# sunilsarolkarcds/ISL-SignLanguage-Translation

Measured on AMD Instinct MI355X. Metric: frames/sec body_25 368×656 fwd+NMS+PAF at 1/8 MI355X; conv MFMA util %, higher is better.
Workload: dtype fp32 (split-fp16 x3 MFMA, fp32 accumulate)

## Files before the change

### isl-signlanguage-translation_amd/csrc/wino_f16.hip

```cpp
#include <algorithm>
#include <cstdlib>
#include <type_traits>

#include "internal.h"

namespace isl {
namespace {

typedef _Float16 f16x8 __attribute__((ext_vector_type(8)));
typedef _Float16 f16x2 __attribute__((ext_vector_type(2)));
typedef float f32x2 __attribute__((ext_vector_type(2)));
typedef float f32x4 __attribute__((ext_vector_type(4)));
typedef float f32x16 __attribute__((ext_vector_type(16)));
typedef unsigned u32x4 __attribute__((ext_vector_type(4)));

struct W2Args {
  const float* in;
  float* out;
  const f16x8* upk;
  const float* bias;
  const float* slope;
  int* range_flag;
  long long in_fs, in_chs, out_fs, out_chs;
  float wscale_inv;
  int in_pad, out_pad, H, W, TH, TW, pairs, cin_chunks, co_blocks, bpf, act, nblocks;
};

constexpr int RS = 34;
constexpr int QS = 6 * 2 * RS;
constexpr int HS = 13 * 64;
constexpr int BUF = 32 * 64;

__device__ __forceinline__ void split_dw(const f32x4& v, unsigned& h01, unsigned& h23, unsigned& l01, unsigned& l23) {
  asm("v_cvt_pk_f16_f32 %0, %1, %2" : "=v"(h01) : "v"(v.x), "v"(v.y));
  asm("v_cvt_pk_f16_f32 %0, %1, %2" : "=v"(h23) : "v"(v.z), "v"(v.w));
  asm("v_fma_mixlo_f16 %0, %1, -1.0, %2 op_sel_hi:[1,0,0]" : "=v"(l01) : "v"(h01), "v"(v.x));
  asm("v_fma_mixhi_f16 %0, %1, -1.0, %2 op_sel:[1,0,0] op_sel_hi:[1,0,0]" : "+v"(l01) : "v"(h01), "v"(v.y));
  asm("v_fma_mixlo_f16 %0, %1, -1.0, %2 op_sel_hi:[1,0,0]" : "=v"(l23) : "v"(h23), "v"(v.z));
  asm("v_fma_mixhi_f16 %0, %1, -1.0, %2 op_sel:[1,0,0] op_sel_hi:[1,0,0]" : "+v"(l23) : "v"(h23), "v"(v.w));
}

template <int ABL>
__global__ void __launch_bounds__(512, 1) wino_f16(W2Args a) {
  __shared__ f32x4 smem[8192 + 32];

  int bid = blockIdx.x;
  {
    const int nb = a.nblocks, q = nb >> 3, r = nb & 7, xcd = bid & 7, k = bid >> 3;
    bid = (xcd < r ? xcd * (q + 1) : r * (q + 1) + (xcd - r) * q) + k;
  }
  const int co_b = bid % a.co_blocks;
  const int rest = bid / a.co_blocks;
  const int fb = rest % a.bpf;
  const int n = rest / a.bpf;

  const int tid = threadIdx.x, lane = tid & 63, h = lane >> 5, l32 = lane & 31;
  const int w = __builtin_amdgcn_readfirstlane(tid >> 6);

  if (tid < 64) {
    float* eb = (float*)(smem + 8192);
    eb[tid] = a.bias[co_b * 64 + tid];
    eb[64 + tid] = a.act == ACT_PRELU ? a.slope[co_b * 64 + tid] : 0.f;
  }

  const int BW = 2 * a.TW, s0 = fb * 64;
  const int ba = s0 / BW, bb = (s0 + 63) / BW;
  const bool two = bb > ba;
  const int txlo0 = (s0 - ba * BW) >> 1;
  const int txhi0 = two ? a.TW - 1 : (s0 + 63 - ba * BW) >> 1;
  const int w0 = 2 * (txhi0 - txlo0 + 1) + 2;
  const int w1 = two ? 2 * (((s0 + 63 - bb * BW) >> 1) + 1) + 2 : 0;
  const int Hp = a.H + 2 * a.in_pad, Wp = a.W + 2 * a.in_pad;
  const float* in_f = a.in + (size_t)n * a.in_fs;

  int doff[4], dch[4];
#pragma unroll
  for (int e = 0; e < 4; ++e) {
    const int p = w + 8 * e;
    const int hp = p < 26 ? p / 13 : 0;
    const int u = (p - 13 * hp) * 64 + lane;
    int t = u / RS;
    const int hc = u - t * RS;
    const int par = t & 1;
    t >>= 1;
    const int row = t % 6;
    const int qq = t / 6;
    const int v = 2 * hc + par;
    const bool s1 = v >= w0;
    const int vl = s1 ? v - w0 : v;
    const bool ok = p < 26 && qq < 2 && vl < (s1 ? w1 : w0);
    const int band = s1 ? bb : ba, txlo = s1 ? 0 : txlo0;
    const int rp = min(4 * band - 1 + row + a.in_pad, Hp - 1);
    const int cp = min(2 * txlo - 1 + vl + a.in_pad, Wp - 1);
    doff[e] = ok ? (rp * Wp + cp) * 8 + qq * 4 : 0;
    dch[e] = __builtin_amdgcn_readfirstlane(hp);
  }

  const int wr = w >> 1, cpr = w & 1;
  const int ra = wr == 0 ? 0 : wr == 2 ? 2 : 1, rb = wr == 3 ? 3 : wr == 2 ? 1 : 2;
  const float sr = wr == 1 ? 1.f : -1.f, sz = cpr ? -1.f : 1.f;
  const f32x4 srv = f32x4{sr, sr, sr, sr}, szv = f32x4{sz, sz, sz, sz};
  const int cX = cpr ? 2 : 0, cY = cpr ? 1 : 2, cZ = cpr ? 3 : 1;
  auto toff = [&](int row, int col) { return (row * 2 + (col & 1)) * RS + (col >> 1); };
  const int to_aX = toff(ra, cX), to_aY = toff(ra, cY), to_aZ = toff(ra, cZ);
  const int to_bX = toff(rb, cX), to_bY = toff(rb, cY), to_bZ = toff(rb, cZ);
  int tb[2];
#pragma unroll
  for (int j = 0; j < 2; ++j) {
    const int s = s0 + 32 * j + l32;
    const int band = s / BW, u = s - band * BW, tx = u >> 1, typ = u & 1;
    const int hc0 = band > ba ? (w0 >> 1) + tx : tx - txlo0;
    tb[j] = h * HS + 2 * typ * 2 * RS + hc0;
  }

  const unsigned uvoff = (unsigned)lane * 16;
  auto load_a = [&](f16x8 (&A)[2][2][2], int k) __attribute__((always_inline)) {
    if constexpr ((ABL & 4) != 0) return;
    const f16x8* u0 = a.upk + ((size_t)(co_b * a.pairs + k) * 16 + 4 * wr + 2 * cpr) * 256;
    const f16x8* u1 = u0 + 256;
    asm volatile(
        "global_load_dwordx4 %0, %8, %9 offset:0\n\t"
        "global_load_dwordx4 %1, %8, %9 offset:1024\n\t"
        "global_load_dwordx4 %2, %8, %9 offset:2048\n\t"
        "global_load_dwordx4 %3, %8, %9 offset:3072\n\t"
        "global_load_dwordx4 %4, %8, %10 offset:0\n\t"
        "global_load_dwordx4 %5, %8, %10 offset:1024\n\t"
        "global_load_dwordx4 %6, %8, %10 offset:2048\n\t"
        "global_load_dwordx4 %7, %8, %10 offset:3072"
        : "=v"(A[0][0][0]), "=v"(A[0][0][1]), "=v"(A[0][1][0]), "=v"(A[0][1][1]), "=v"(A[1][0][0]),
          "=v"(A[1][0][1]), "=v"(A[1][1][0]), "=v"(A[1][1][1])
        : "v"(uvoff), "s"(u0), "s"(u1)
        : "memory");
  };
  auto dma = [&](int k, int sl) __attribute__((always_inline)) {
    if constexpr ((ABL & 8) != 0) return;
#pragma unroll
    for (int e = 0; e < 4; ++e) {
      const int ch = min(2 * k + dch[e], a.cin_chunks - 1);
      const float* src = in_f + (size_t)ch * a.in_chs;
      __builtin_amdgcn_global_load_lds((const void*)(src + doff[e]),
                                       (__attribute__((address_space(3))) void*)(smem + sl * BUF + (w + 8 * e) * 64),
                                       16, 0, 0);
    }
  };

  f32x16 acc[2][2][2];
#pragma unroll
  for (int x = 0; x < 2; ++x)
#pragma unroll
    for (int i = 0; i < 2; ++i)
#pragma unroll
      for (int j = 0; j < 2; ++j)
#pragma unroll
        for (int r = 0; r < 16; ++r) acc[x][i][j][r] = 0.f;

  auto compute = [&](const f16x8 (&A)[2][2][2], int sl) __attribute__((always_inline)) {
#pragma unroll
    for (int j = 0; j < 2; ++j) {
      int b = tb[j] + sl * BUF;
      asm volatile("" : "+v"(b));
      unsigned Bd[2][2][4];
      if constexpr ((ABL & 2) != 0) {
#pragma unroll
        for (int x = 0; x < 2; ++x)
#pragma unroll
          for (int hl = 0; hl < 2; ++hl)
#pragma unroll
            for (int d = 0; d < 4; ++d) Bd[x][hl][d] = 0x3c003c00u;
      } else {
        auto quad = [&](auto qc) __attribute__((always_inline)) {
          constexpr int Q = decltype(qc)::value;
          const f32x4 aX = smem[b + to_aX + Q * QS], aY = smem[b + to_aY + Q * QS], aZ = smem[b + to_aZ + Q * QS];
          const f32x4 bX = smem[b + to_bX + Q * QS], bY = smem[b + to_bY + Q * QS], bZ = smem[b + to_bZ + Q * QS];
          const f32x4 tX = __builtin_elementwise_fma(srv, bX, aX);
          const f32x4 tY = __builtin_elementwise_fma(srv, bY, aY);
          const f32x4 tZ = __builtin_elementwise_fma(srv, bZ, aZ);
          const f32x4 v0 = tX - tY;
          const f32x4 v1 = __builtin_elementwise_fma(szv, tZ, tY);
          split_dw(v0, Bd[0][0][2 * Q], Bd[0][0][2 * Q + 1], Bd[0][1][2 * Q], Bd[0][1][2 * Q + 1]);
          split_dw(v1, Bd[1][0][2 * Q], Bd[1][0][2 * Q + 1], Bd[1][1][2 * Q], Bd[1][1][2 * Q + 1]);
        };
        quad(std::integral_constant<int, 0>{});
        quad(std::integral_constant<int, 1>{});
      }
      f16x8 Bh[2], Bl[2];
#pragma unroll
      for (int x = 0; x < 2; ++x) {
        Bh[x] = __builtin_bit_cast(f16x8, u32x4{Bd[x][0][0], Bd[x][0][1], Bd[x][0][2], Bd[x][0][3]});
        Bl[x] = __builtin_bit_cast(f16x8, u32x4{Bd[x][1][0], Bd[x][1][1], Bd[x][1][2], Bd[x][1][3]});
      }
#pragma unroll
      for (int x = 0; x < 2; ++x)
#pragma unroll
        for (int i = 0; i < 2; ++i) {
          if constexpr ((ABL & 1) != 0) continue;
          acc[x][i][j] = __builtin_amdgcn_mfma_f32_32x32x16_f16(A[x][i][0], Bh[x], acc[x][i][j], 0, 0, 0);
          acc[x][i][j] = __builtin_amdgcn_mfma_f32_32x32x16_f16(A[x][i][0], Bl[x], acc[x][i][j], 0, 0, 0);
          acc[x][i][j] = __builtin_amdgcn_mfma_f32_32x32x16_f16(A[x][i][1], Bh[x], acc[x][i][j], 0, 0, 0);
        }
    }
  };

  f16x8 AS[2][2][2][2];
  load_a(AS[0], 0);
  dma(0, 0);
  dma(min(1, a.pairs - 1), 1);
  asm volatile("s_waitcnt vmcnt(4)" ::: "memory");
  __syncthreads();
  __builtin_amdgcn_sched_barrier(0);
  auto step = [&](int k, f16x8 (&A)[2][2][2], f16x8 (&An)[2][2][2]) __attribute__((always_inline)) {
    load_a(An, min(k + 1, a.pairs - 1));
    dma(min(k + 2, a.pairs - 1), (k + 2) % 3);
    __builtin_amdgcn_sched_barrier(0);
    if constexpr ((ABL & 4) == 0)
      asm volatile("s_waitcnt vmcnt(16)"
                   : "+v"(A[0][0][0]), "+v"(A[0][0][1]), "+v"(A[0][1][0]), "+v"(A[0][1][1]), "+v"(A[1][0][0]),
                     "+v"(A[1][0][1]), "+v"(A[1][1][0]), "+v"(A[1][1][1])
                   :
                   : "memory");
    compute(A, k % 3);
    __builtin_amdgcn_sched_barrier(0);
    asm volatile("s_waitcnt vmcnt(12) lgkmcnt(0)" ::: "memory");
    __builtin_amdgcn_s_barrier();
    __builtin_amdgcn_sched_barrier(0);
  };
  for (int k = 0; k < a.pairs; k += 2) {
    step(k, AS[0], AS[1]);
    if (k + 1 < a.pairs) step(k + 1, AS[1], AS[0]);
  }
  asm volatile("s_waitcnt vmcnt(0) lgkmcnt(0)"
               : "+v"(AS[0][0][0][0]), "+v"(AS[0][0][0][1]), "+v"(AS[0][0][1][0]), "+v"(AS[0][0][1][1]),
                 "+v"(AS[0][1][0][0]), "+v"(AS[0][1][0][1]), "+v"(AS[0][1][1][0]), "+v"(AS[0][1][1][1]),
                 "+v"(AS[1][0][0][0]), "+v"(AS[1][0][0][1]), "+v"(AS[1][0][1][0]), "+v"(AS[1][0][1][1]),
                 "+v"(AS[1][1][0][0]), "+v"(AS[1][1][0][1]), "+v"(AS[1][1][1][0]), "+v"(AS[1][1][1][1])
               :
               : "memory");
  __syncthreads();

  bool bad = false;
  if constexpr ((ABL & 16) != 0) {
    float sum = 0.f;
#pragma unroll
    for (int x = 0; x < 2; ++x)
#pragma unroll
      for (int i = 0; i < 2; ++i)
#pragma unroll
        for (int j = 0; j < 2; ++j)
#pragma unroll
          for (int r = 0; r < 16; ++r) sum += acc[x][i][j][r];
    if (sum == 1.2345f || bad) atomicOr(a.range_flag, 1);
    return;
  }
  f32x4* xm = smem;
  const float* eb = (const float*)(smem + 8192);
  const int Wo = a.W + 2 * a.out_pad;
  float* out_f = a.out + (size_t)n * a.out_fs;
  const int rn = tid & 31, rh = (tid >> 5) & 1, rq = (tid >> 6) & 3, rj = tid >> 8;
  const int rs = s0 + 32 * rj + rn, rband = rs / BW, ru = rs - rband * BW, rtx = ru >> 1, rty = 2 * rband + (ru & 1);
#pragma unroll
  for (int i = 0; i < 2; ++i) {
#pragma unroll
    for (int x = 0; x < 2; ++x)
#pragma unroll
      for (int j = 0; j < 2; ++j)
#pragma unroll
        for (int q = 0; q < 4; ++q)
          xm[((((2 * w + x) * 2 + j) * 4 + q) * 2 + h) * 32 + l32] =
              f32x4{acc[x][i][j][4 * q], acc[x][i][j][4 * q + 1], acc[x][i][j][4 * q + 2], acc[x][i][j][4 * q + 3]};
    __syncthreads();
    {
      const f32x4* mp = xm + ((rj * 4 + rq) * 2 + rh) * 32 + rn;
      f32x4 R0[4], R1[4];
#pragma unroll
      for (int c = 0; c < 4; ++c) {
        const f32x4 m0 = mp[(0 + c) * 512], m1 = mp[(4 + c) * 512], m2 = mp[(8 + c) * 512], m3 = mp[(12 + c) * 512];
        R0[c] = (m0 + m1) + m2;
        R1[c] = (m1 - m2) - m3;
      }
      f32x4 Y[2][2];
      Y[0][0] = (R0[0] + R0[1]) + R0[2];
      Y[0][1] = (R0[1] - R0[2]) - R0[3];
      Y[1][0] = (R1[0] + R1[1]) + R1[2];
      Y[1][1] = (R1[1] - R1[2]) - R1[3];
      const int cl = i * 32 + 8 * rq + 4 * rh, co = co_b * 64 + cl;
      const f32x4 bv = *(const f32x4*)(eb + cl);
      const f32x4 sl = *(const f32x4*)(eb + 64 + cl);
      if (rty < a.TH) {
        float* oc = out_f + (size_t)(co >> 3) * a.out_chs + (co & 7);
#pragma unroll
        for (int yy = 0; yy < 2; ++yy)
#pragma unroll
          for (int xx = 0; xx < 2; ++xx) {
            const int y = 2 * rty + yy, x = 2 * rtx + xx;
            if (y >= a.H || x >= a.W) continue;
            f32x4 v;
#pragma unroll
            for (int e = 0; e < 4; ++e) v[e] = Y[yy][xx][e] * a.wscale_inv + bv[e];
            if (a.act == ACT_RELU) {
#pragma unroll
              for (int e = 0; e < 4; ++e) v[e] = v[e] > 0.f ? v[e] : 0.f;
            } else if (a.act == ACT_PRELU) {
#pragma unroll
              for (int e = 0; e < 4; ++e) v[e] = v[e] >= 0.f ? v[e] : v[e] * sl[e];
            }
#pragma unroll
            for (int e = 0; e < 4; ++e) bad |= !(__builtin_fabsf(v[e]) < 65504.f);
            *(f32x4*)(oc + (size_t)((y + a.out_pad) * Wo + x + a.out_pad) * 8) = v;
          }
      }
    }
    __syncthreads();
  }
  if (bad) atomicOr(a.range_flag, 1);
}

int g_wino_blocks(const ConvLaunch& c, int* bpf) {
  const int TH = (c.H + 1) / 2, TW = (c.W + 1) / 2, nbands = (TH + 1) / 2;
  *bpf = (nbands * 2 * TW + 63) / 64;
  return c.n * *bpf * (c.cout / 64);
}

}

bool wino_f16_fits(const ConvLaunch& c) {
  return c.ks == 3 && c.in_pad >= 1 && c.cout % 64 == 0 && c.cout > 0 && !c.hpool && !c.vin && !c.fold &&
         c.cout7 == 0 && (c.W + 1) / 2 >= 32 && (long long)c.H * c.W > 1024 &&
         !((c.in_cs | c.in_coff | c.out_cs | c.out_coff) & 7) && (long long)(c.H + 2 * c.in_pad) * (c.W + 2 * c.in_pad) * 8 < (1ll << 30);
}

hipError_t launch_wino_f16(const ConvLaunch& c, hipStream_t s) {
  if (!wino_f16_fits(c)) { set_error("wino_f16: launch not eligible"); return hipErrorInvalidValue; }
  if (!c.wx3 || !c.range_flag) { set_error("wino_f16: split filters / range flag missing"); return hipErrorInvalidValue; }
  W2Args a{};
  a.in_chs = (long long)(c.H + 2 * c.in_pad) * (c.W + 2 * c.in_pad) * 8;
  a.out_chs = (long long)(c.H + 2 * c.out_pad) * (c.W + 2 * c.out_pad) * 8;
  a.in_fs = a.in_chs * (c.in_cs / 8);
  a.out_fs = a.out_chs * (c.out_cs / 8);
  a.in = c.in + (c.in_coff / 8) * a.in_chs;
  a.out = c.out + (c.out_coff / 8) * a.out_chs;
  a.upk = (const f16x8*)c.wx3;
  a.bias = c.bias;
  a.slope = c.slope;
  a.range_flag = c.range_flag;
  a.wscale_inv = c.wscale_inv;
  a.in_pad = c.in_pad;
  a.out_pad = c.out_pad;
  a.H = c.H;
  a.W = c.W;
  a.TH = (c.H + 1) / 2;
  a.TW = (c.W + 1) / 2;
  a.pairs = (c.cin_chunks + 1) / 2;
  a.cin_chunks = c.cin_chunks;
  a.co_blocks = c.cout / 64;
  a.act = c.act;
  const long long nb = g_wino_blocks(c, &a.bpf);
  if (nb <= 0 || nb > 0x7fffffff) { set_error("wino_f16: bad grid"); return hipErrorInvalidValue; }
  a.nblocks = (int)nb;
#ifdef ISLPOSE_DEV
  const int abl = getenv("ISLPOSE_W2_ABL") ? atoi(getenv("ISLPOSE_W2_ABL")) : 0;
  switch (abl) {
#define W2ABL(k) case k: hipLaunchKernelGGL(wino_f16<k>, dim3(a.nblocks), dim3(512), 0, s, a); return hipGetLastError();
    W2ABL(1) W2ABL(2) W2ABL(3) W2ABL(4) W2ABL(6) W2ABL(8) W2ABL(12) W2ABL(14) W2ABL(16) W2ABL(31)
#undef W2ABL
    default: break;
  }
#endif
  hipLaunchKernelGGL(wino_f16<0>, dim3(a.nblocks), dim3(512), 0, s, a);
  return hipGetLastError();
}

double wino_f16_mfma_flops(const ConvLaunch& c) {
  int bpf = 0;
  const double nb = g_wino_blocks(c, &bpf);
  return nb * 16.0 * 64 * 64 * 16.0 * ((c.cin_chunks + 1) / 2) * 2 * 3;
}

}
```

Measured before the change: 1291.

## Software-pipeline LDS reads of Winograd input tiles ahead of transform and MFMA

Adds a prefetching compute path that issues the ds_read_b128 loads for the next quad/column group through inline asm before the current group's input transform and MFMAs run. The first group's reads are hoisted to the start of each step, ahead of the global loads. The B-transform now uses packed v_pk_fma_f32 with scalar sign constants, and the DMA offsets become byte offsets. The goal is to hide LDS latency behind the arithmetic, at the cost of more registers and hand-placed waitcnt barriers that could stall or cause hazards. The prefetch variant becomes the default, and the old path stays reachable through an env var in dev builds.

```diff
diff --git a/isl-signlanguage-translation_amd/csrc/wino_f16.hip b/isl-signlanguage-translation_amd/csrc/wino_f16.hip
--- a/isl-signlanguage-translation_amd/csrc/wino_f16.hip
+++ b/isl-signlanguage-translation_amd/csrc/wino_f16.hip
@@ -40,7 +40,18 @@
   asm("v_fma_mixhi_f16 %0, %1, -1.0, %2 op_sel:[1,0,0] op_sel_hi:[1,0,0]" : "+v"(l23) : "v"(h23), "v"(v.w));
 }
 
-template <int ABL>
+struct W2Raw {
+  f32x4 aX, aY, aZ, bX, bY, bZ;
+};
+__device__ __forceinline__ f32x2 pk_fma_s(unsigned long long s, f32x2 b, f32x2 a) {
+  f32x2 d;
+  asm("v_pk_fma_f32 %0, %1, %2, %3" : "=v"(d) : "s"(s), "v"(b), "v"(a));
+  return d;
+}
+__device__ __forceinline__ f32x2 lo2(const f32x4& v) { return f32x2{v.x, v.y}; }
+__device__ __forceinline__ f32x2 hi2(const f32x4& v) { return f32x2{v.z, v.w}; }
+
+template <int ABL, int PF>
 __global__ void __launch_bounds__(512, 1) wino_f16(W2Args a) {
   __shared__ f32x4 smem[8192 + 32];
 
@@ -73,7 +84,8 @@
   const int Hp = a.H + 2 * a.in_pad, Wp = a.W + 2 * a.in_pad;
   const float* in_f = a.in + (size_t)n * a.in_fs;
 
-  int doff[4], dch[4];
+  unsigned doff[4];
+  int dch[4];
 #pragma unroll
   for (int e = 0; e < 4; ++e) {
     const int p = w + 8 * e;
@@ -92,7 +104,7 @@
     const int band = s1 ? bb : ba, txlo = s1 ? 0 : txlo0;
     const int rp = min(4 * band - 1 + row + a.in_pad, Hp - 1);
     const int cp = min(2 * txlo - 1 + vl + a.in_pad, Wp - 1);
-    doff[e] = ok ? (rp * Wp + cp) * 8 + qq * 4 : 0;
+    doff[e] = ok ? (unsigned)((rp * Wp + cp) * 8 + qq * 4) * 4u : 0u;
     dch[e] = __builtin_amdgcn_readfirstlane(hp);
   }
 
@@ -100,6 +112,10 @@
   const int ra = wr == 0 ? 0 : wr == 2 ? 2 : 1, rb = wr == 3 ? 3 : wr == 2 ? 1 : 2;
   const float sr = wr == 1 ? 1.f : -1.f, sz = cpr ? -1.f : 1.f;
   const f32x4 srv = f32x4{sr, sr, sr, sr}, szv = f32x4{sz, sz, sz, sz};
+  const unsigned sru = __builtin_amdgcn_readfirstlane(__builtin_bit_cast(unsigned, sr));
+  const unsigned szu = __builtin_amdgcn_readfirstlane(__builtin_bit_cast(unsigned, sz));
+  const unsigned long long sr2 = (unsigned long long)sru << 32 | sru, sz2 = (unsigned long long)szu << 32 | szu;
+  const unsigned lds0 = (unsigned)(__UINTPTR_TYPE__)(__attribute__((address_space(3))) void*)smem;
   const int cX = cpr ? 2 : 0, cY = cpr ? 1 : 2, cZ = cpr ? 3 : 1;
   auto toff = [&](int row, int col) { return (row * 2 + (col & 1)) * RS + (col >> 1); };
   const int to_aX = toff(ra, cX), to_aY = toff(ra, cY), to_aZ = toff(ra, cZ);
@@ -138,7 +154,9 @@
     for (int e = 0; e < 4; ++e) {
       const int ch = min(2 * k + dch[e], a.cin_chunks - 1);
       const float* src = in_f + (size_t)ch * a.in_chs;
-      __builtin_amdgcn_global_load_lds((const void*)(src + doff[e]),
+      unsigned d = doff[e];
+      asm volatile("" : "+v"(d));
+      __builtin_amdgcn_global_load_lds((const void*)((const char*)src + (size_t)d),
                                        (__attribute__((address_space(3))) void*)(smem + sl * BUF + (w + 8 * e) * 64),
                                        16, 0, 0);
     }
@@ -153,6 +171,96 @@
       for (int j = 0; j < 2; ++j)
 #pragma unroll
         for (int r = 0; r < 16; ++r) acc[x][i][j][r] = 0.f;
+
+  const unsigned oaX = lds0 + 16 * to_aX, oaY = lds0 + 16 * to_aY, oaZ = lds0 + 16 * to_aZ;
+  const unsigned obX = lds0 + 16 * to_bX, obY = lds0 + 16 * to_bY, obZ = lds0 + 16 * to_bZ;
+  auto rd = [&](W2Raw& r, int sl, int j, auto qc, f32x2* t) __attribute__((always_inline)) {
+    constexpr int OFF = decltype(qc)::value * QS * 16;
+    if constexpr ((ABL & 32) != 0) {
+      asm volatile("" : "=v"(r.aX), "=v"(r.bX), "=v"(r.aY), "=v"(r.bY), "=v"(r.aZ), "=v"(r.bZ));
+      return;
+    }
+    unsigned b = (unsigned)(tb[j] + sl * BUF) * 16;
+    asm volatile("" : "+v"(b));
+    const unsigned paX = b + oaX, paY = b + oaY, paZ = b + oaZ, pbX = b + obX, pbY = b + obY, pbZ = b + obZ;
+#define W2_READS                           \
+  "ds_read_b128 %0, %6 offset:%12\n\t"     \
+  "ds_read_b128 %1, %7 offset:%12\n\t"     \
+  "ds_read_b128 %2, %8 offset:%12\n\t"     \
+  "ds_read_b128 %3, %9 offset:%12\n\t"     \
+  "ds_read_b128 %4, %10 offset:%12\n\t"    \
+  "ds_read_b128 %5, %11 offset:%12"
+    if (t)
+      asm volatile(W2_READS
+                   : "=&v"(r.aX), "=&v"(r.bX), "=&v"(r.aY), "=&v"(r.bY), "=&v"(r.aZ), "=&v"(r.bZ)
+                   : "v"(paX), "v"(pbX), "v"(paY), "v"(pbY), "v"(paZ), "v"(pbZ), "n"(OFF), "v"(t[0]), "v"(t[1]),
+                     "v"(t[2]), "v"(t[3]), "v"(t[4]), "v"(t[5])
+                   : "memory");
+    else
+      asm volatile(W2_READS
+                   : "=&v"(r.aX), "=&v"(r.bX), "=&v"(r.aY), "=&v"(r.bY), "=&v"(r.aZ), "=&v"(r.bZ)
+                   : "v"(paX), "v"(pbX), "v"(paY), "v"(pbY), "v"(paZ), "v"(pbZ), "n"(OFF)
+                   : "memory");
+#undef W2_READS
+  };
+  auto compute_pf = [&](const f16x8 (&A)[2][2][2], int sl, W2Raw r) __attribute__((always_inline)) {
+    unsigned Bd[2][2][4];
+    auto group = [&](auto jc, auto qc) __attribute__((always_inline)) {
+      constexpr int j = decltype(jc)::value, Q = decltype(qc)::value;
+      if constexpr ((ABL & 32) != 0) {
+      } else if constexpr (j == 0 && Q == 0) {
+        asm volatile("s_waitcnt lgkmcnt(0)"
+                     : "+v"(r.aX), "+v"(r.bX), "+v"(r.aY), "+v"(r.bY), "+v"(r.aZ), "+v"(r.bZ)
+                     :
+                     : "memory");
+      } else if constexpr (Q == 1) {
+        asm volatile("s_waitcnt lgkmcnt(0)"
+                     : "+v"(r.aX), "+v"(r.bX), "+v"(r.aY), "+v"(r.bY), "+v"(r.aZ), "+v"(r.bZ), "+v"(Bd[0][0][0]),
+                       "+v"(Bd[0][0][1]), "+v"(Bd[0][1][0]), "+v"(Bd[0][1][1]), "+v"(Bd[1][0][0]), "+v"(Bd[1][0][1]),
+                       "+v"(Bd[1][1][0]), "+v"(Bd[1][1][1])
+                     :
+                     : "memory");
+      } else {
+        asm volatile("s_waitcnt lgkmcnt(0)"
+                     : "+v"(r.aX), "+v"(r.bX), "+v"(r.aY), "+v"(r.bY), "+v"(r.aZ), "+v"(r.bZ), "+v"(acc[0][0][0]),
+                       "+v"(acc[0][1][0])
+                     :
+                     : "memory");
+      }
+      f32x2 t[6];
+      t[0] = pk_fma_s(sr2, lo2(r.bX), lo2(r.aX)), t[1] = pk_fma_s(sr2, hi2(r.bX), hi2(r.aX));
+      t[2] = pk_fma_s(sr2, lo2(r.bY), lo2(r.aY)), t[3] = pk_fma_s(sr2, hi2(r.bY), hi2(r.aY));
+      t[4] = pk_fma_s(sr2, lo2(r.bZ), lo2(r.aZ)), t[5] = pk_fma_s(sr2, hi2(r.bZ), hi2(r.aZ));
+      if constexpr (Q == 0) rd(r, sl, j, std::integral_constant<int, 1>{}, t);
+      else if constexpr (j == 0) rd(r, sl, 1, std::integral_constant<int, 0>{}, t);
+      if constexpr (j == 0 || Q == 0) __builtin_amdgcn_sched_barrier(0);
+      const f32x2 v00 = t[0] - t[2], v01 = t[1] - t[3];
+      const f32x2 v10 = pk_fma_s(sz2, t[4], t[2]), v11 = pk_fma_s(sz2, t[5], t[3]);
+      split_dw(f32x4{v00.x, v00.y, v01.x, v01.y}, Bd[0][0][2 * Q], Bd[0][0][2 * Q + 1], Bd[0][1][2 * Q], Bd[0][1][2 * Q + 1]);
+      split_dw(f32x4{v10.x, v10.y, v11.x, v11.y}, Bd[1][0][2 * Q], Bd[1][0][2 * Q + 1], Bd[1][1][2 * Q], Bd[1][1][2 * Q + 1]);
+      if constexpr (Q == 1) {
+        f16x8 Bh[2], Bl[2];
+#pragma unroll
+        for (int x = 0; x < 2; ++x) {
+          Bh[x] = __builtin_bit_cast(f16x8, u32x4{Bd[x][0][0], Bd[x][0][1], Bd[x][0][2], Bd[x][0][3]});
+          Bl[x] = __builtin_bit_cast(f16x8, u32x4{Bd[x][1][0], Bd[x][1][1], Bd[x][1][2], Bd[x][1][3]});
+        }
+#pragma unroll
+        for (int x = 0; x < 2; ++x)
+#pragma unroll
+          for (int i = 0; i < 2; ++i) {
+            if constexpr ((ABL & 1) != 0) continue;
+            acc[x][i][j] = __builtin_amdgcn_mfma_f32_32x32x16_f16(A[x][i][0], Bh[x], acc[x][i][j], 0, 0, 0);
+            acc[x][i][j] = __builtin_amdgcn_mfma_f32_32x32x16_f16(A[x][i][0], Bl[x], acc[x][i][j], 0, 0, 0);
+            acc[x][i][j] = __builtin_amdgcn_mfma_f32_32x32x16_f16(A[x][i][1], Bh[x], acc[x][i][j], 0, 0, 0);
+          }
+      }
+    };
+    group(std::integral_constant<int, 0>{}, std::integral_constant<int, 0>{});
+    group(std::integral_constant<int, 0>{}, std::integral_constant<int, 1>{});
+    group(std::integral_constant<int, 1>{}, std::integral_constant<int, 0>{});
+    group(std::integral_constant<int, 1>{}, std::integral_constant<int, 1>{});
+  };
 
   auto compute = [&](const f16x8 (&A)[2][2][2], int sl) __attribute__((always_inline)) {
 #pragma unroll
@@ -209,6 +317,8 @@
   __syncthreads();
   __builtin_amdgcn_sched_barrier(0);
   auto step = [&](int k, f16x8 (&A)[2][2][2], f16x8 (&An)[2][2][2]) __attribute__((always_inline)) {
+    W2Raw r0;
+    if constexpr (PF != 0) rd(r0, k % 3, 0, std::integral_constant<int, 0>{}, nullptr);
     load_a(An, min(k + 1, a.pairs - 1));
     dma(min(k + 2, a.pairs - 1), (k + 2) % 3);
     __builtin_amdgcn_sched_barrier(0);
@@ -218,7 +328,8 @@
                      "+v"(A[1][0][1]), "+v"(A[1][1][0]), "+v"(A[1][1][1])
                    :
                    : "memory");
-    compute(A, k % 3);
+    if constexpr (PF != 0) compute_pf(A, k % 3, r0);
+    else compute(A, k % 3);
     __builtin_amdgcn_sched_barrier(0);
     asm volatile("s_waitcnt vmcnt(12) lgkmcnt(0)" ::: "memory");
     __builtin_amdgcn_s_barrier();
@@ -359,13 +470,23 @@
 #ifdef ISLPOSE_DEV
   const int abl = getenv("ISLPOSE_W2_ABL") ? atoi(getenv("ISLPOSE_W2_ABL")) : 0;
   switch (abl) {
-#define W2ABL(k) case k: hipLaunchKernelGGL(wino_f16<k>, dim3(a.nblocks), dim3(512), 0, s, a); return hipGetLastError();
+#define W2ABL(k) case k: hipLaunchKernelGGL((wino_f16<k, 0>), dim3(a.nblocks), dim3(512), 0, s, a); return hipGetLastError();
     W2ABL(1) W2ABL(2) W2ABL(3) W2ABL(4) W2ABL(6) W2ABL(8) W2ABL(12) W2ABL(14) W2ABL(16) W2ABL(31)
 #undef W2ABL
+    case 65: hipLaunchKernelGGL((wino_f16<1, 1>), dim3(a.nblocks), dim3(512), 0, s, a); return hipGetLastError();
+    case 68: hipLaunchKernelGGL((wino_f16<4, 1>), dim3(a.nblocks), dim3(512), 0, s, a); return hipGetLastError();
+    case 72: hipLaunchKernelGGL((wino_f16<8, 1>), dim3(a.nblocks), dim3(512), 0, s, a); return hipGetLastError();
+    case 76: hipLaunchKernelGGL((wino_f16<12, 1>), dim3(a.nblocks), dim3(512), 0, s, a); return hipGetLastError();
+    case 80: hipLaunchKernelGGL((wino_f16<16, 1>), dim3(a.nblocks), dim3(512), 0, s, a); return hipGetLastError();
+    case 32: hipLaunchKernelGGL((wino_f16<32, 1>), dim3(a.nblocks), dim3(512), 0, s, a); return hipGetLastError();
     default: break;
   }
+  if (getenv("ISLPOSE_W2_PF") && atoi(getenv("ISLPOSE_W2_PF")) == 0) {
+    hipLaunchKernelGGL((wino_f16<0, 0>), dim3(a.nblocks), dim3(512), 0, s, a);
+    return hipGetLastError();
+  }
 #endif
-  hipLaunchKernelGGL(wino_f16<0>, dim3(a.nblocks), dim3(512), 0, s, a);
+  hipLaunchKernelGGL((wino_f16<0, 1>), dim3(a.nblocks), dim3(512), 0, s, a);
   return hipGetLastError();
 }
 
```

After: 1313 (median of 6 runs). 1.7% higher.
